# Thraix/VoxelRayTracer

Measured on AMD Instinct MI355X. Metric: Mrays/sec + achieved HBM GB/s, 1920x1080 @ 128^3 voxels, 4 bounces, higher is better.
Workload: dtype f32

## Files before the change

### voxelraytracer_amd/csrc/vrt_render.hip

```cpp
#include <hip/hip_ext.h>
#include <hip/hip_runtime.h>

#include <algorithm>
#include <cmath>
#include <cstdint>
#include <cstdio>
#include <cstring>
#include <string>
#include <vector>

#include "vrt.h"
#include "vrt_internal.h"
#include "vrt_diag.h"
#include "vrt_math.h"
#include "vrt_walk.h"
#include "vrt_cert.h"
#include "vrt_aux_kernels.h"
#include "vrt_skipfield_kernels.h"

namespace vrt {

__device__ __forceinline__ uint32_t unorm8(float f) {
  const float c = __builtin_fminf(__builtin_fmaxf(f, 0.0f), 1.0f);
  return uint32_t(__builtin_rintf(c * 255.0f));
}
__device__ __forceinline__ float unorm8_read(uint32_t b) {
  const float a = float(b), y = 1.0f / 255.0f;
  const float q0 = a * y;
  return __builtin_fmaf(__builtin_fmaf(-255.0f, q0, a), y, q0);
}
__device__ __forceinline__ uint32_t pack_rgb8(float r, float g, float b) {
  return unorm8(r) | (unorm8(g) << 8) | (unorm8(b) << 16) | 0xFF000000u;
}
__device__ __forceinline__ uint32_t temporal_blend(uint32_t nw, uint32_t old, float alpha) {
  const float om = 1.0f - alpha;
  uint32_t r = 0xFF000000u;
#pragma unroll
  for (int ch = 0; ch < 3; ++ch) {
    const float v = alpha * unorm8_read((nw >> (8 * ch)) & 0xFFu) + om * unorm8_read((old >> (8 * ch)) & 0xFFu);
    r |= unorm8(v) << (8 * ch);
  }
  return r;
}

__device__ __forceinline__ uint32_t lane_id() {
  uint32_t l;
  asm volatile("v_mbcnt_lo_u32_b32 %0, -1, 0\n\tv_mbcnt_hi_u32_b32 %0, -1, %0" : "=v"(l));
  return l;
}

__device__ __forceinline__ uint32_t* ord_ctr(const KArgs& a, uint32_t set, uint32_t r) {
  return a.order + (set * kOrdClasses + r) * kOrdCtrStride;
}
__device__ __forceinline__ uint32_t* ord_rank(const KArgs& a, uint32_t set) {
  return a.order + kOrdHdr + (1u + set) * a.tiles;
}
__device__ __forceinline__ uint32_t* ord_list(const KArgs& a, uint32_t set) {
  return a.order + kOrdHdr + 3u * a.tiles + set * (a.tiles + kOrdClasses);
}
__device__ __forceinline__ uint32_t ordered_tile(const KArgs& a, uint32_t L) {
  const uint32_t cap = kOrdClasses * a.ord_q;
  if (L < cap) {
    const uint32_t r = L % kOrdClasses, j = L / kOrdClasses;
    if (j == 0u && threadIdx.x == 0u) *ord_ctr(a, a.ctr_z, r) = 0u;
    const uint32_t n = min(*ord_ctr(a, a.ctr_r, r), a.ord_q);
    return j < n ? ord_list(a, a.ord_r)[(n - 1u - j) * kOrdClasses + r] : ~0u;
  }
  const uint32_t t = L - cap;
  return ord_rank(a, a.ord_r)[t] - 1u < a.ord_q ? ~0u : t;
}
__device__ __forceinline__ void order_record(const KArgs& a, uint32_t tile, bool heavy_wave) {
  uint32_t* cnt = a.order + kOrdHdr + tile;
  const uint32_t add = 1u | (heavy_wave ? 0x100u : 0u);
  const uint32_t old = atomicAdd(cnt, add);
  if ((old & 0xFFu) != uint32_t(kWgWaves) - 1u) return;
  *cnt = 0u;
  uint32_t rank = 0u;
  if (((old + add) & 0xFF00u) != 0u) {
    const uint32_t r = tile % kOrdClasses;
    const uint32_t k = atomicAdd(ord_ctr(a, a.ctr_w, r), 1u);
    ord_list(a, a.ord_w)[k * kOrdClasses + r] = tile;
    rank = k + 1u;
  }
  ord_rank(a, a.ord_w)[tile] = rank;
}

__device__ __forceinline__ int pixel_x(uint32_t tx, int wave, uint32_t lane) {
  return int(tx) * kTileW + (wave & 1) * 8 + int(lane & 7u);
}
__device__ __forceinline__ int pixel_row(uint32_t ty, int wave, uint32_t lane) {
  return int(ty) * kTileH + (wave >> 1) * 8 + int(lane >> 3);
}
__device__ __forceinline__ int frame_row(const KArgs& a, int li) {
  return a.row0 + (li >> a.row_blk_sh) * a.row_step + (li & ((1 << a.row_blk_sh) - 1));
}


struct FrameView {
  const float* pv;
  float time;
  uint32_t* cur;
  uint32_t* raw;
};
__device__ __forceinline__ FrameView frame_view(const KArgs& a, uint32_t f) {
  if (f == 0u) return FrameView{a.inv_pv, a.time, a.cur, a.raw};
  const KArgs::FrameB& b = a.fb[f - 1u];
  return FrameView{b.inv_pv, b.time, b.cur, b.raw};
}

template <bool LATE = false>
__device__ __forceinline__ void init_ctx(Ctx& c, const KArgs& a, const uint16_t* __restrict__ vox) {
  c.vox = vox;
  c.ostride = a.ostride;
  c.n = a.n;
  c.p = uint32_t(a.n) + 1u;
  c.fn = a.fn;
  c.max_len = a.max_len;
  c.time = a.time;
  c.refl_noise = a.refl_noise;
  c.refr_noise = a.refr_noise;
  if constexpr (LATE) {
    c.sky_sy = 0.0f;
    c.sun_n = c.sun_rcp = mk(0.0f, 0.0f, 0.0f);
    c.atlas = nullptr;
    c.atlas_mask = 0u;
    c.atlas_fs = c.atlas_fts = 0.0f;
  } else {
    c.sky_sy = a.sky_sy;
    c.sun_n = mk(a.sun_n[0], a.sun_n[1], a.sun_n[2]);
    c.sun_rcp = mk(a.sun_rcp[0], a.sun_rcp[1], a.sun_rcp[2]);
    c.atlas = a.atlas;
    c.atlas_mask = uint32_t(a.atlas_size) - 1u;
    c.atlas_fs = float(a.atlas_size);
    c.atlas_fts = float(a.atlas_tex_size);
  }
  CTRACE_ONLY(c.tr = false;)
}

__device__ __forceinline__ bool markstein_safe(float x) {
  const float m = __builtin_fabsf(x);
  return m >= 0x1p-60f && m <= 0x1p60f;
}
__device__ __forceinline__ f3 div3_rn(float x, float y, float z, float d) {
  if (markstein_safe(x) && markstein_safe(y) && markstein_safe(z) && markstein_safe(d)) {
    const float r = rcp_newton(d);
    return mk(div_rn(x, d, r), div_rn(y, d, r), div_rn(z, d, r));
  }
  return mk(x / d, y / d, z / d);
}
__device__ __forceinline__ f3 div3_lean(float x, float y, float z, float d, float r, bool rest) {
  const bool safe = rest & (__builtin_fminf(__builtin_fminf(__builtin_fabsf(x), __builtin_fabsf(y)), __builtin_fabsf(z)) >=
                            0x1p-60f);
  if (safe) return mk(div_rn(x, d, r), div_rn(y, d, r), div_rn(z, d, r));
  return mk(x / d, y / d, z / d);
}
__device__ __forceinline__ bool div3_lean_ranges(float x, float y, float z, float d) {
  return int(__builtin_fabsf(x) <= 0x1p60f) & int(__builtin_fabsf(y) <= 0x1p60f) & int(__builtin_fabsf(z) <= 0x1p60f) &
         int(markstein_safe(d));
}

template <bool LEAN = false>
__device__ __forceinline__ Ray primary_ray(const KArgs& a, const float* __restrict__ inv_pv, const Ctx& c, int px,
                                           int py) {
  const float ndx = div_rn(2.0f * (float(px) + 0.5f), LEAN ? a.fw : float(a.width), a.rcp_w) - 1.0f;
  const float ndy = div_rn(2.0f * (float(py) + 0.5f), LEAN ? a.fh : float(a.height), a.rcp_h) - 1.0f;
  float n4[4], f4[4];
#pragma unroll
  for (int i = 0; i < (LEAN ? 3 : 4); ++i) {
    const float base = inv_pv[0 * 4 + i] * ndx + inv_pv[1 * 4 + i] * ndy;
    n4[i] = (base + inv_pv[2 * 4 + i] * -1.0f) + inv_pv[3 * 4 + i] * 1.0f;
    f4[i] = (base + inv_pv[2 * 4 + i] * 1.0f) + inv_pv[3 * 4 + i] * 1.0f;
  }
  f3 vnear, vdir;
  if constexpr (LEAN) {
    float rn, rf;
    bool rest_n = true, rest_f = true;
    if ((a.setup & kSetupW) != 0u) {
      n4[3] = a.wn;
      f4[3] = a.wf;
      rn = a.rcp_wn;
      rf = a.rcp_wf;
    } else {
      const float base = inv_pv[0 * 4 + 3] * ndx + inv_pv[1 * 4 + 3] * ndy;
      n4[3] = (base + inv_pv[2 * 4 + 3] * -1.0f) + inv_pv[3 * 4 + 3] * 1.0f;
      f4[3] = (base + inv_pv[2 * 4 + 3] * 1.0f) + inv_pv[3 * 4 + 3] * 1.0f;
      if (a.vdiv_ok == 0u) {
        rest_n = div3_lean_ranges(n4[0], n4[1], n4[2], n4[3]);
        rest_f = div3_lean_ranges(f4[0], f4[1], f4[2], f4[3]);
      }
      rn = rcp_newton(n4[3]);
      rf = rcp_newton(f4[3]);
    }
    vnear = div3_lean(n4[0], n4[1], n4[2], n4[3], rn, rest_n);
    vdir = div3_lean(f4[0], f4[1], f4[2], f4[3], rf, rest_f) - vnear;
  } else {
    vnear = div3_rn(n4[0], n4[1], n4[2], n4[3]);
    vdir = div3_rn(f4[0], f4[1], f4[2], f4[3]) - vnear;
  }
  Ray ray;
  const float half_n = LEAN ? a.half_n : c.fn * 0.5f;
  ray.pos = mk(vnear.x + half_n, vnear.y + half_n, vnear.z + half_n);
  f3 dir0;
  if constexpr (LEAN) {
    const float s = vdir.x * vdir.x + vdir.y * vdir.y + vdir.z * vdir.z;
    float inv;
    if ((a.setup & kSetupLen) != 0u)
      inv = rcp_newton(sqrt_fix(s));
    else
      inv = normalize3_scale(s);
    dir0 = vdir * inv;
  } else {
    dir0 = normalize3(vdir);
  }
  ray.dir = randomize<LEAN>(dir0, vnear, a.ray_noise, c.time);
  ray.len = 0.0f;
  ray.energy = 1.0f;
  ray.voxel = 0;
  ray.rdepth = 0;
  ray.tdepth = 0;
  return ray;
}

constexpr int kStackPrio = 3;

struct StackRay {
  f3 pos, dir;
  float len, energy;
  uint32_t depths;
};
__device__ __forceinline__ StackRay pack_stack_ray(const Ray& r) {
  return StackRay{r.pos, r.dir, r.len, r.energy, uint32_t(r.rdepth) | (uint32_t(r.tdepth) << 16)};
}
constexpr int kStackWords = 9;
template <int NL>
__device__ __forceinline__ void lds_stack_put(float* __restrict__ b, const StackRay& e) {
  b[0 * NL] = e.pos.x;
  b[1 * NL] = e.pos.y;
  b[2 * NL] = e.pos.z;
  b[3 * NL] = e.dir.x;
  b[4 * NL] = e.dir.y;
  b[5 * NL] = e.dir.z;
  b[6 * NL] = e.len;
  b[7 * NL] = e.energy;
  b[8 * NL] = __uint_as_float(e.depths);
}
template <int NL>
__device__ __forceinline__ StackRay lds_stack_get(const float* __restrict__ b) {
  return StackRay{mk(b[0 * NL], b[1 * NL], b[2 * NL]), mk(b[3 * NL], b[4 * NL], b[5 * NL]), b[6 * NL],
                  b[7 * NL], __float_as_uint(b[8 * NL])};
}
__device__ __forceinline__ Ray unpack_stack_ray(const StackRay& e) {
  Ray r;
  r.pos = e.pos;
  r.dir = e.dir;
  r.len = e.len;
  r.energy = e.energy;
  r.voxel = 0;
  r.rdepth = int32_t(e.depths & 0xffffu);
  r.tdepth = int32_t(e.depths >> 16);
  return r;
}

template <bool STATS, bool TEX, bool CSH = false, bool CSEC = false, int NL = kWgThreads>
__device__ __forceinline__ bool exact_pixel(const KArgs& a, const Ctx& c, Ray ray, f3& color,
                                            Counters& k, uint32_t& steps, uint32_t& flags,
                                            int32_t& hit_vidx, float& hit_len, float* __restrict__ lstk,
                                            float s_init = -1.0f) {
  StackRay stack[kMaxStack - 2];
  const int cap = a.max_refl + a.max_transp + 1;
  int sp = 0;
  const Hit h0 = trace_with_shadow<STATS, TEX, true, CSH>(c, ray, color, k, steps, flags, s_init);
  STAMP_PIXEL_BEGIN();
  hit_vidx = h0.found ? h0.vidx : -1;
  hit_len = h0.found ? h0.len : 0.0f;
  if (h0.found && mat_id(h0.voxel) == 2) {
    __builtin_amdgcn_s_setprio(kStackPrio);
    Hit h = h0;
    for (;;) {
      Ctx lc = c;
      asm volatile("" : "+s"(lc.sun_n.x), "+s"(lc.sun_n.y), "+s"(lc.sun_n.z), "+s"(lc.sun_rcp.x),
                   "+s"(lc.sun_rcp.y), "+s"(lc.sun_rcp.z));
      bool push_r = false, push_t = false;
      if (h.found) {
        const uint32_t m = mat_id(h.voxel);
        const bool pr = mat_reflective(m) && ray.rdepth < a.max_refl;
        const bool pt = mat_transparent(m) && ray.tdepth < a.max_transp && get_color<TEX>(lc, h).w != 1.0f;
        push_r = pr && sp < cap;
        push_t = pt && sp + int(push_r) < cap;
        if ((pr && !push_r) || (pt && !push_t)) flags |= VRT_HIT_FLAG_STACK_FULL;
      }
      if (push_r && push_t) {
        const StackRay e = pack_stack_ray(reflection_ray(lc, ray, h));
        if (sp == 0)
          lds_stack_put<NL>(lstk, e);
        else
          stack[sp - 1] = e;
        ++sp;
        ray = refraction_ray<TEX>(lc, ray, h, k);
      } else if (push_r) {
        ray = reflection_ray(lc, ray, h);
      } else if (push_t) {
        ray = refraction_ray<TEX>(lc, ray, h, k);
      } else {
        if (sp == 0) break;
        --sp;
        ray = unpack_stack_ray(sp == 0 ? lds_stack_get<NL>(lstk) : stack[sp - 1]);
      }
      k.c[VRT_CNT_SECONDARY_RAYS]++;
      if constexpr (CSH && CSEC) {
        bool settled;
        h = march_cert(lc, ray, color, settled, k, steps, flags);
        if (settled) {
          h.found = false;
          continue;
        }
        shade<STATS, TEX, CSH>(lc, ray, h, color, k, steps, flags);
        continue;
      }
      h = trace_with_shadow<STATS, TEX, false, CSH>(lc, ray, color, k, steps, flags);
    }
    STAMP_PIXEL_END();
    return true;
  }
  return false;
}

template <class KA>
__device__ __forceinline__ void store_pixel(const KA& a, const FrameView& fv, float4* __restrict__ out,
                                            size_t o, const f3 color) {
  if (fv.cur) {
    const uint32_t rw = pack_rgb8(color.x, color.y, color.z);
    if (fv.raw) fv.raw[o] = rw;
    fv.cur[o] = a.alpha == 1.0f ? rw : temporal_blend(rw, a.prev[o], a.alpha);
  } else {
    out[o] = make_float4(color.x, color.y, color.z, 1.0f);
  }
}

template <bool STATS, bool TEX, int CERT = 0, bool ORD = false, bool DEFER = false, bool FB = false,
          bool TREE = false>
__global__ void __launch_bounds__(kWgThreads, TREE ? kTreeWaves : (DEFER ? kDeferWaves : kMinWaves)) render_kernel(KArgs a, const uint16_t* __restrict__ vox,
                                                     float4* __restrict__ out,
                                                     vrt_hit* __restrict__ hits,
                                                     unsigned long long* __restrict__ counters) {
  const int wave = __builtin_amdgcn_readfirstlane(int(threadIdx.x) >> 6);
  STAMP_WAVE_BEGIN(wave);
  uint32_t tile = 0u;
  uint32_t fr = 0u, tx, ty;
  if constexpr (DEFER) {
    static_assert(!ORD, "the certified pass has no tile order");
    tx = blockIdx.x;
    ty = blockIdx.y;
    if constexpr (FB) fr = blockIdx.z;
  } else {
    tile = blockIdx.x;
    if constexpr (ORD) {
      tile = ordered_tile(a, blockIdx.x);
      if (tile == ~0u) return;
    }
    tile = __builtin_amdgcn_readfirstlane(tile);
    if constexpr (FB) fr = uint32_t(__builtin_amdgcn_readfirstlane(int(tile / a.frame_tiles)));
    const uint32_t ltile = tile - fr * a.frame_tiles;
    ty = ltile / a.tiles_x;
    tx = ltile - ty * a.tiles_x;
  }
  const int px = pixel_x(tx, wave, lane_id());
  const int li = pixel_row(ty, wave, lane_id());
  const bool valid = px < a.width && li < a.rows;
  bool heavy = false;
  bool deferred = false;

  Counters k;
#pragma unroll
  for (int q = 0; q < VRT_CNT_COUNT; ++q) k.c[q] = 0;

  if (valid) {
    Ctx c;
    init_ctx<DEFER>(c, a, vox);
    CTRACE_ONLY(c.tr = px == VRT_TRACE_PX && frame_row(a, li) == VRT_TRACE_PY;)
    if constexpr (FB) c.time = frame_view(a, fr).time;
    constexpr int kAxFloats = DEFER && !TREE ? 0 : kWgThreads * 3 * 4;
    constexpr int kStkFloats = std::max(DEFER ? 0 : kStackWords * kWgThreads,
                                        TREE ? (kTreeWords - 12) * kWgThreads : 0);
    constexpr int kPool = std::max(kAxFloats + kStkFloats, 4);
    __shared__ float4 lds_pool[kPool / 4];
    c.ax = &lds_pool[threadIdx.x * kAxLane];
    const Ray ray = primary_ray<DEFER>(a, FB ? frame_view(a, fr).pv : a.inv_pv, c, px, frame_row(a, li));
    k.c[VRT_CNT_PIXELS] = 1;
    k.c[VRT_CNT_PRIMARY_RAYS] = 1;
    uint32_t steps = 0, flags = 0;
    int32_t hit_vidx = -1;
    float hit_len = 0.0f;
    f3 color;
    if constexpr (!DEFER) color = mk(0.0f, 0.0f, 0.0f);
    float* tstk = nullptr;
    if constexpr (TREE) {
      static_assert(CERT == 2 && !TEX && !STATS, "certified trees: stats-free colour-only certified instances");
      tstk = reinterpret_cast<float*>(lds_pool) + kAxFloats + threadIdx.x;
    }
    float us = -1.0f;
    bool need_exact;
    if (DEFER && (PHASE_STOP(0) || PHASE_STOP(1))) {
      color = PHASE_STOP(1) ? mk(ray.pos.x + ray.dir.x, ray.pos.y + ray.dir.y, ray.pos.z + ray.dir.z)
                            : mk(0.0f, 0.0f, 0.0f);
      need_exact = false;
    } else {
      need_exact = CERT < 2 || !cert_pixel<TEX, TREE, kWgThreads, DEFER>(c, ray, color, a.max_refl, a.max_transp, tstk, &us, &a);
    }
    STAMP_WAVE_CERT(need_exact);
    if constexpr (DEFER) {
      deferred = need_exact;
    } else if (need_exact) {
      color = mk(0.0f, 0.0f, 0.0f);
      heavy = true;
      float* lstk = reinterpret_cast<float*>(lds_pool) + kAxFloats;
      (void)exact_pixel<STATS, TEX, CERT >= 1, CERT == 2>(a, c, ray, color, k, steps, flags, hit_vidx,
                                                         hit_len, &lstk[threadIdx.x], STATS ? -1.0f : us);
    }
    const uint32_t l2 = lane_id();
    const size_t o = size_t(pixel_row(ty, wave, l2)) * size_t(a.pitch) + size_t(pixel_x(tx, wave, l2));
    if (STATS && hits) {
      vrt_hit hr;
      hr.voxel_index = hit_vidx;
      hr.ray_length = hit_len;
      hr.steps = steps;
      hr.flags = flags;
      hits[o] = hr;
    }
    if constexpr (DEFER) {
      if (!deferred) {
        LateKArgs* ka = late_kargs();
        uint32_t *cur = ka->cur, *raw = ka->raw;
        if (FB && fr != 0u) {
          cur = ka->fb[fr - 1u].cur;
          raw = ka->fb[fr - 1u].raw;
        }
        store_pixel(*ka, FrameView{nullptr, 0.0f, cur, raw}, out, o, color);
      }
    } else {
      if (!deferred) store_pixel(a, FB ? frame_view(a, fr) : FrameView{a.inv_pv, a.time, a.cur, a.raw}, out, o, color);
    }
  }
  if constexpr (DEFER) {
    const unsigned long long m = __ballot(deferred);
    if (m != 0ull) {
      const uint32_t seg = tx * kOrdClasses / a.tiles_x;
      const uint32_t first = uint32_t(__builtin_ctzll(m));
      const uint32_t cnt = uint32_t(__builtin_popcountll(m));
      const bool dense = cnt >= kDeferDense;
      uint32_t base = 0;
      if (lane_id() == first)
        base = atomicAdd(a.defer + ((uint32_t(dense) * 2u + a.defer_e) * kOrdClasses + seg) * kOrdCtrStride,
                         dense ? 1u : cnt);
      base = uint32_t(__builtin_amdgcn_readlane(int(base), int(first)));
      uint32_t* list = a.defer + kDeferHdr + seg * a.defer_seg;
      const uint32_t l3 = lane_id();
      const uint32_t id = (fr << 29) | (uint32_t(pixel_row(ty, wave, l3)) << 16) | uint32_t(pixel_x(tx, wave, l3));
      if (dense) {
        list[a.defer_seg - 64u * (base + 1u) + l3] = deferred ? id : ~0u;
      } else if (deferred) {
        const uint32_t rank = __builtin_amdgcn_mbcnt_hi(uint32_t(m >> 32), __builtin_amdgcn_mbcnt_lo(uint32_t(m), 0u));
        list[base + rank] = id;
      }
    }
  }
  if constexpr (ORD) {
    const bool heavy_wave = __ballot(heavy) != 0ull;
    if (lane_id() == 0) order_record(a, tile, heavy_wave);
  }
  STAMP_WAVE_END();
  if (STATS && counters) {
    unsigned long long* slot = counters + size_t(blockIdx.x % kCntReplicas) * VRT_CNT_COUNT;
#pragma unroll
    for (int q = 0; q < VRT_CNT_COUNT; ++q) {
      unsigned long long v = k.c[q];
#pragma unroll
      for (int off = 32; off > 0; off >>= 1) v += __shfl_xor(v, off, 64);
      if (lane_id() == 0 && v) atomicAdd(slot + q, v);
    }
  }
}

template <bool TEX, int CERT, int WAVES = kExactWaves, uint32_t SB = kSparseBatch, bool FB = false>
__global__ void __launch_bounds__(64, WAVES) exact_pass_kernel(KArgs a, const uint16_t* __restrict__ vox,
                                                                     float4* __restrict__ out) {
  const uint32_t* ctr = a.defer;
  if (blockIdx.x == 0 && threadIdx.x < 2u * kOrdClasses) {
    const uint32_t l = threadIdx.x;
    a.defer[(((l / kOrdClasses) * 2u + (a.defer_e ^ 1u)) * kOrdClasses + l % kOrdClasses) * kOrdCtrStride] = 0u;
  }
  uint32_t ns[kOrdClasses], nd[kOrdClasses], total_s = 0, total_d = 0;
#pragma unroll
  for (uint32_t q = 0; q < kOrdClasses; ++q) {
    ns[q] = uint32_t(__builtin_amdgcn_readfirstlane(int(ctr[(a.defer_e * kOrdClasses + q) * kOrdCtrStride])));
    nd[q] = uint32_t(__builtin_amdgcn_readfirstlane(int(ctr[((2u + a.defer_e) * kOrdClasses + q) * kOrdCtrStride])));
    total_s += ns[q];
    total_d += nd[q];
  }
  static_assert(SB >= 1 && SB <= 64, "lanes SB.. of a sparse batch idle");
  const uint32_t batches = total_d + (total_s + SB - 1u) / SB;
  if (a.batches_out && blockIdx.x == 0 && threadIdx.x == 0)
    *a.batches_out = batches;
  if (blockIdx.x >= batches) return;
  if constexpr (kExactPrio > 0) __builtin_amdgcn_s_setprio(kExactPrio);
  const uint32_t lane = lane_id();
  STAMP_PASS_BEGIN();
  Ctx c;
  init_ctx(c, a, vox);
  __shared__ float4 ax_tab[64 * 3];
  c.ax = &ax_tab[lane * kAxLane];
  for (uint32_t b = blockIdx.x; b < batches; b += gridDim.x) {
    const bool dense = b < total_d;
    uint32_t idx = dense ? b : (b - total_d) * SB + lane;
    if (!dense && (lane >= SB || idx >= total_s)) continue;
    uint32_t seg = 0;
#pragma unroll
    for (uint32_t q = 0; q + 1u < kOrdClasses; ++q) {
      const uint32_t nq = dense ? nd[q] : ns[q];
      const bool past = seg == q && idx >= nq;
      idx -= past ? nq : 0u;
      seg += past ? 1u : 0u;
    }
    const uint32_t* list = a.defer + kDeferHdr + seg * a.defer_seg;
    const uint32_t e = dense ? list[a.defer_seg - 64u * (idx + 1u) + lane] : list[idx];
    if (e == ~0u) continue;
    Ray ray;
    if constexpr (FB) {
      const FrameView fv = frame_view(a, e >> 29);
      c.time = fv.time;
      ray = primary_ray(a, fv.pv, c, int(e & 0xFFFFu), frame_row(a, int((e >> 16) & 0x1FFFu)));
    } else {
      ray = primary_ray(a, a.inv_pv, c, int(e & 0xFFFFu), frame_row(a, int(e >> 16)));
    }
    Counters k;
#pragma unroll
    for (int q = 0; q < VRT_CNT_COUNT; ++q) k.c[q] = 0;
    uint32_t steps = 0, flags = 0;
    int32_t hit_vidx = -1;
    float hit_len = 0.0f;
    f3 color = mk(0.0f, 0.0f, 0.0f);
    __shared__ float lstk[kStackWords * 64];
    (void)exact_pixel<false, TEX, CERT >= 1, CERT == 2 && !TEX, 64>(a, c, ray, color, k, steps, flags,
                                                                    hit_vidx, hit_len, &lstk[lane]);
    if constexpr (FB) {
      uint32_t e2 = e;
      asm volatile("" : "+v"(e2));
      store_pixel(a, frame_view(a, e2 >> 29), out,
                  size_t((e2 >> 16) & 0x1FFFu) * size_t(a.pitch) + size_t(e2 & 0xFFFFu), color);
    } else {
      store_pixel(a, FrameView{a.inv_pv, a.time, a.cur, a.raw}, out,
                  size_t(e >> 16) * size_t(a.pitch) + size_t(e & 0xFFFFu), color);
    }
    STAMP_PASS_BATCH(dense);
  }
  STAMP_PASS_END(lane);
}

}

#include "vrt_query_kernels.h"
#include "vrt_trace_kernels.h"
#include "vrt_ids_kernels.h"
#include "vrt_reproject_kernels.h"

namespace vrt {


static unsigned grid_blocks(uint64_t items) { return unsigned(std::min<uint64_t>((items + 255) / 256, 16384)); }

void launch_render(const KArgs& a, bool stats, const uint16_t* vox, float4* out, vrt_hit* hit,
                   unsigned long long* cnt_rep, hipStream_t s, hipEvent_t ev_begin, hipEvent_t ev_end) {
  const dim3 grid(a.order ? kOrdClasses * a.ord_q + a.tiles : a.tiles);
  if (a.defer && !stats && a.cert == 2) {
    const dim3 g1(a.tiles_x, a.frame_tiles / a.tiles_x, uint32_t(a.nframes)),
        g2(a.exact_grid ? a.exact_grid
                        : std::max(64u, a.tiles * uint32_t(kWgWaves) / (a.textured ? kDeferGridDiv : kDeferGridDivColor)));
    const bool fb = a.nframes > 1;
    auto k1 = a.textured ? (fb ? render_kernel<false, true, 2, false, true, true> : render_kernel<false, true, 2, false, true>)
              : a.tree   ? (fb ? render_kernel<false, false, 2, false, true, true, true>
                               : render_kernel<false, false, 2, false, true, false, true>)
                         : (fb ? render_kernel<false, false, 2, false, true, true> : render_kernel<false, false, 2, false, true>);
    auto k2 = a.textured ? (fb ? exact_pass_kernel<true, 1, kExactWaves, kSparseBatchTex, true>
                               : exact_pass_kernel<true, 1, kExactWaves, kSparseBatchTex>)
                         : (a.exact_fat
                                ? (fb ? exact_pass_kernel<false, 2, kFatWaves, kSparseBatchFat, true>
                                      : exact_pass_kernel<false, 2, kFatWaves, kSparseBatchFat>)
                                : (fb ? exact_pass_kernel<false, 2, kExactWaves, kSparseBatch, true>
                                      : exact_pass_kernel<false, 2>));
    const uint32_t pad = a.tree ? 0u : kDeferLdsPad;
    if (ev_begin)
      hipExtLaunchKernelGGL(k1, g1, dim3(kWgThreads), pad, s, ev_begin, nullptr, 0, a, vox, out, hit, cnt_rep);
    else
      hipLaunchKernelGGL(k1, g1, dim3(kWgThreads), pad, s, a, vox, out, hit, cnt_rep);
    if (ev_end)
      hipExtLaunchKernelGGL(k2, g2, dim3(64), 0, s, nullptr, ev_end, 0, a, vox, out);
    else
      hipLaunchKernelGGL(k2, g2, dim3(64), 0, s, a, vox, out);
    return;
  }
  auto kern = a.textured ? (stats ? render_kernel<true, true>
                            : a.nframes > 1 ? (a.cert >= 1 ? render_kernel<false, true, 1, false, false, true>
                                                           : render_kernel<false, true, 0, false, false, true>)
                                            : (a.cert >= 1 ? render_kernel<false, true, 1> : render_kernel<false, true>))
                         : (stats ? render_kernel<true, false>
                            : a.nframes > 1
                                ? (a.cert == 2 ? (a.order ? render_kernel<false, false, 2, true, false, true>
                                                          : render_kernel<false, false, 2, false, false, true>)
                                   : a.cert == 1 ? render_kernel<false, false, 1, false, false, true>
                                                 : render_kernel<false, false, 0, false, false, true>)
                                : (a.cert == 2 ? (a.tree ? (a.order ? render_kernel<false, false, 2, true, false, false, true>
                                                                    : render_kernel<false, false, 2, false, false, false, true>)
                                                 : a.order ? render_kernel<false, false, 2, true>
                                                           : render_kernel<false, false, 2>)
                                   : a.cert == 1 ? render_kernel<false, false, 1>
                                                 : render_kernel<false, false, 0>));
  if (ev_begin || ev_end)
    hipExtLaunchKernelGGL(kern, grid, dim3(kWgThreads), 0, s, ev_begin, ev_end, 0, a, vox, out, hit, cnt_rep);
  else
    hipLaunchKernelGGL(kern, grid, dim3(kWgThreads), 0, s, a, vox, out, hit, cnt_rep);
}

void launch_ray_query(const KArgs& a, int32_t kind, const uint16_t* vox, const void* in, uint32_t count,
                      vrt_ray_hit* hits, hipStream_t s, hipEvent_t ev_begin, hipEvent_t ev_end) {
  auto kern = kind == kQueryPick           ? ray_query_kernel<kQueryPick>
              : kind == VRT_CAST_OCCLUSION ? ray_query_kernel<VRT_CAST_OCCLUSION>
                                           : ray_query_kernel<VRT_CAST_NEAREST>;
  const dim3 grid((count + uint32_t(kQueryWg) - 1u) / uint32_t(kQueryWg));
  if (ev_begin || ev_end)
    hipExtLaunchKernelGGL(kern, grid, dim3(kQueryWg), 0, s, ev_begin, ev_end, 0, a, vox, in, count,
                          reinterpret_cast<uint4*>(hits));
  else
    hipLaunchKernelGGL(kern, grid, dim3(kQueryWg), 0, s, a, vox, in, count, reinterpret_cast<uint4*>(hits));
}

void launch_ray_trace(const KArgs& a, int32_t kind, const uint16_t* vox, const void* in, uint32_t count,
                      vrt_ray_color* out, hipStream_t s, hipEvent_t ev_begin, hipEvent_t ev_end) {
  auto kern = kind == kTracePixels
                  ? (a.textured ? ray_trace_kernel<kTracePixels, true> : ray_trace_kernel<kTracePixels, false>)
                  : (a.textured ? ray_trace_kernel<kTraceRays, true> : ray_trace_kernel<kTraceRays, false>);
  const dim3 grid((count + uint32_t(kTraceWg) - 1u) / uint32_t(kTraceWg));
  if (ev_begin || ev_end)
    hipExtLaunchKernelGGL(kern, grid, dim3(kTraceWg), 0, s, ev_begin, ev_end, 0, a, vox, in, count,
                          reinterpret_cast<uint4*>(out));
  else
    hipLaunchKernelGGL(kern, grid, dim3(kTraceWg), 0, s, a, vox, in, count, reinterpret_cast<uint4*>(out));
}

void launch_render_ids(const KArgs& a, const uint16_t* vox, vrt_pixel_id* ids, float* depth, hipStream_t s,
                       hipEvent_t ev_begin, hipEvent_t ev_end) {
  const dim3 grid(uint32_t(a.width + 7) / 8u, uint32_t(a.rows + 7) / 8u);
  if (ev_begin || ev_end)
    hipExtLaunchKernelGGL(ids_exact_kernel, grid, dim3(64), 0, s, ev_begin, ev_end, 0, a, vox,
                          reinterpret_cast<uint2*>(ids), depth);
  else
    hipLaunchKernelGGL(ids_exact_kernel, grid, dim3(64), 0, s, a, vox, reinterpret_cast<uint2*>(ids), depth);
}

void launch_reproject(const KArgs& a, const ReprojArgs& r, hipStream_t s, hipEvent_t ev_begin, hipEvent_t ev_end) {
  const dim3 grid(uint32_t(a.width + 15) / 16u, uint32_t(a.rows + 15) / 16u);
  if (ev_begin || ev_end)
    hipExtLaunchKernelGGL(reproject_kernel, grid, dim3(kReprojWg), 0, s, ev_begin, ev_end, 0, a, r);
  else
    hipLaunchKernelGGL(reproject_kernel, grid, dim3(kReprojWg), 0, s, a, r);
}

void launch_reproject_fetch(const KArgs& a, const ReprojArgs& r, int32_t fetch, uint8_t* taps, hipStream_t s,
                            hipEvent_t ev_begin, hipEvent_t ev_end) {
  if (fetch == VRT_FETCH_NEAREST && !taps) return launch_reproject(a, r, s, ev_begin, ev_end);
  auto kern = fetch == VRT_FETCH_BILINEAR ? reproject_bilinear_kernel : reproject_nearest_taps_kernel;
  const dim3 grid(uint32_t(a.width + 15) / 16u, uint32_t(a.rows + 15) / 16u);
  if (ev_begin || ev_end)
    hipExtLaunchKernelGGL(kern, grid, dim3(kReprojWg), 0, s, ev_begin, ev_end, 0, a, r, taps);
  else
    hipLaunchKernelGGL(kern, grid, dim3(kReprojWg), 0, s, a, r, taps);
}

void launch_reduce_counters(unsigned long long* rep, unsigned long long* dst, hipStream_t s) {
  hipLaunchKernelGGL(reduce_counters_kernel, dim3(1), dim3(64), 0, s, rep, dst);
}

namespace {

struct Span {
  int32_t a, b;
};
Span clip_span(int64_t a, int64_t b, int32_t n) {
  return Span{int32_t(std::max<int64_t>(a, 0)), int32_t(std::min<int64_t>(b, int64_t(n) - 1))};
}
Span fwd_anchors(int32_t lo, int32_t hi, int sg, int32_t n) {
  const int64_t r = int64_t(kFwdCap) - 1;
  return sg > 0 ? clip_span(lo - r, int64_t(hi) - 1, n) : clip_span(lo, int64_t(hi) - 1 + r, n);
}
Span fwd_inputs(int32_t lo, int32_t hi, int32_t n) {
  const int64_t r = int64_t(kFwdCap) - 1;
  return clip_span(lo - r, int64_t(hi) - 1 + r, n);
}
Span fwd_texels(int32_t lo, int32_t hi, int sg, int32_t n) {
  const int64_t r = int64_t(kFwdCap) - 1;
  const int64_t a = (sg > 0 ? lo - r : int64_t(lo)) + sg, b = (sg > 0 ? int64_t(hi) - 1 : int64_t(hi) - 1 + r) + sg;
  return clip_span(std::min<int64_t>(a, lo), std::max<int64_t>(b, int64_t(hi) - 1), n);
}
Span dist_span(int32_t lo, int32_t hi, int64_t reach, int32_t n) {
  return clip_span(lo - reach, int64_t(hi) - 1 + reach, n);
}
Region region_of(Span x, Span y, Span z) {
  return Region{x.a, y.a, z.a, x.b - x.a + 1, y.b - y.a + 1, z.b - z.a + 1};
}

}

int volume_edit_plan(int32_t n, int octants, const int32_t lo[3], const int32_t ext[3], int32_t* out) {
  for (int o = 0; o < octants; ++o)
    for (int a = 0; a < 3; ++a) {
      const int32_t hi = lo[a] + ext[a];
      const Span t = octants == 8 ? fwd_texels(lo[a], hi, (o >> a & 1) ? -1 : 1, n)
                                  : dist_span(lo[a], hi, int64_t(kDistCap) - 1, n);
      out[o * 6 + a] = t.a;
      out[o * 6 + 3 + a] = t.b + 1;
    }
  return octants;
}

void launch_edit_apply(const uint8_t* box, uint8_t* vox, uint32_t n, const int32_t lo[3], const int32_t ext[3],
                       unsigned long long* counts, hipStream_t s) {
  const Region b{lo[0], lo[1], lo[2], ext[0], ext[1], ext[2]};
  hipLaunchKernelGGL(edit_apply_kernel, dim3(grid_blocks(region_cells(b))), dim3(256), 0, s, box, vox, b, n,
                     counts);
}

void launch_volume_edit_passes(const uint8_t* vox, uint8_t* tmp, uint16_t* packed, uint32_t n, int octants,
                               const int32_t lo[3], const int32_t ext[3], bool distances, hipStream_t s) {
  const int32_t ni = int32_t(n);
  const int32_t hi[3] = {lo[0] + ext[0], lo[1] + ext[1], lo[2] + ext[2]};
  const uint64_t vol = uint64_t(n) * n * n, pvol = uint64_t(n + 1) * (n + 1) * (n + 1);
  const Region box{lo[0], lo[1], lo[2], ext[0], ext[1], ext[2]};
  const Region whole{0, 0, 0, ni, ni, ni};
  uint8_t* da = tmp;
  uint8_t* db = tmp + vol;
  if (octants == 8) {
    uint8_t* dc = tmp + 2 * vol;
    const Span iy = fwd_inputs(lo[1], hi[1], ni), iz = fwd_inputs(lo[2], hi[2], ni);
    for (int sx = 1; sx >= -1; sx -= 2) {
      const Span ax = fwd_anchors(lo[0], hi[0], sx, ni);
      const Region rx = region_of(ax, iy, iz);
      if (distances)
        hipLaunchKernelGGL(fwd_pass_kernel, dim3(grid_blocks(region_cells(rx))), dim3(256), 0, s, vox,
                           whole, da, rx, n, 0, sx, 1);
      for (int sy = 1; sy >= -1; sy -= 2) {
        const Span ay = fwd_anchors(lo[1], hi[1], sy, ni);
        const Region ry = region_of(ax, ay, iz);
        if (distances)
          hipLaunchKernelGGL(fwd_pass_kernel, dim3(grid_blocks(region_cells(ry))), dim3(256), 0, s, da,
                             rx, db, ry, n, 1, sy, 0);
        for (int sz = 1; sz >= -1; sz -= 2) {
          const Span az = fwd_anchors(lo[2], hi[2], sz, ni);
          const Region rz = region_of(ax, ay, az);
          const int o = (sx < 0 ? 1 : 0) | (sy < 0 ? 2 : 0) | (sz < 0 ? 4 : 0);
          uint16_t* dst = packed + size_t(o) * pvol;
          if (distances) {
            hipLaunchKernelGGL(fwd_pass_kernel, dim3(grid_blocks(region_cells(rz))), dim3(256), 0, s, db,
                               ry, dc, rz, n, 2, sz, 0);
            const Region pb = region_of(fwd_texels(lo[0], hi[0], sx, ni), fwd_texels(lo[1], hi[1], sy, ni),
                                        fwd_texels(lo[2], hi[2], sz, ni));
            hipLaunchKernelGGL(fwd_pack_kernel, dim3(grid_blocks(region_cells(pb))), dim3(256), 0, s, vox,
                               dc, rz, dst, pb, n, sx, sy, sz);
          } else {
            hipLaunchKernelGGL(fwd_pack_kernel, dim3(grid_blocks(region_cells(box))), dim3(256), 0, s, vox,
                               static_cast<const uint8_t*>(nullptr), box, dst, box, n, sx, sy, sz);
          }
        }
      }
    }
  } else if (distances) {
    const int64_t r1 = int64_t(kDistCap) - 1;
    const Span ax = dist_span(lo[0], hi[0], r1, ni), ay = dist_span(lo[1], hi[1], r1, ni);
    const Span az = dist_span(lo[2], hi[2], r1, ni);
    const Span iy = dist_span(lo[1], hi[1], 2 * r1, ni), iz = dist_span(lo[2], hi[2], 2 * r1, ni);
    const Region rx = region_of(ax, iy, iz), ry = region_of(ax, ay, iz), rz = region_of(ax, ay, az);
    hipLaunchKernelGGL(dist_pass_kernel, dim3(grid_blocks(region_cells(rx))), dim3(256), 0, s, vox, whole,
                       da, rx, n, 0, 1);
    hipLaunchKernelGGL(dist_pass_kernel, dim3(grid_blocks(region_cells(ry))), dim3(256), 0, s, da, rx, db,
                       ry, n, 1, 0);
    hipLaunchKernelGGL(dist_pass_kernel, dim3(grid_blocks(region_cells(rz))), dim3(256), 0, s, db, ry, da,
                       rz, n, 2, 0);
    hipLaunchKernelGGL(pack_volume_kernel, dim3(grid_blocks(region_cells(rz))), dim3(256), 0, s, vox, da,
                       rz, packed, rz, n);
  } else {
    hipLaunchKernelGGL(pack_volume_kernel, dim3(grid_blocks(region_cells(box))), dim3(256), 0, s, vox,
                       static_cast<const uint8_t*>(nullptr), box, packed, box, n);
  }
  const int wrap = (lo[0] == 0 ? 1 : 0) | (lo[1] == 0 ? 2 : 0) | (lo[2] == 0 ? 4 : 0);
  if (wrap) {
    const EdgeSlabs e = edge_slabs(box, wrap);
    hipLaunchKernelGGL(edge_pack_kernel, dim3(grid_blocks(e.cz + e.cy + e.cx)), dim3(256), 0, s, vox, packed, pvol,
                       octants, box, wrap, n);
  }
}

void launch_glass_share(const uint8_t* vox, uint64_t total, unsigned long long* out, hipStream_t s) {
  hipLaunchKernelGGL(glass_share_kernel, dim3(grid_blocks(total)), dim3(256), 0, s, vox, total, out);
}

void launch_build_scene(uint8_t* vox, int scene, uint32_t n, const float* noise, hipStream_t s) {
  const uint64_t vol = uint64_t(n) * n * n;
  hipLaunchKernelGGL(build_scene_kernel, dim3(grid_blocks(vol)), dim3(256), 0, s, vox, scene, n, noise);
}

void launch_assemble_blocks(const uint32_t* bands, uint64_t band_words, int32_t k, int32_t sh, int32_t width,
                            int32_t height, uint32_t* frame, uint64_t frame_pitch, hipStream_t s) {
  if (height <= 0 || width <= 0) return;
  const bool vec = width % 4 == 0 && band_words % 4 == 0 && frame_pitch % 4 == 0 &&
                   (reinterpret_cast<uintptr_t>(bands) & 15u) == 0 && (reinterpret_cast<uintptr_t>(frame) & 15u) == 0;
  if (vec)
    hipLaunchKernelGGL(assemble_blocks_kernel<true>, dim3(uint32_t(height)), dim3(256), 0, s, bands, band_words, k,
                       sh, width, frame, frame_pitch);
  else
    hipLaunchKernelGGL(assemble_blocks_kernel<false>, dim3(uint32_t(height)), dim3(256), 0, s, bands, band_words, k,
                       sh, width, frame, frame_pitch);
}

void launch_pack_rgb8(const uint32_t* rgba, uint64_t pixels, uint8_t* rgb, hipStream_t s) {
  const uint64_t quads = pixels / 4u;
  if (quads == 0) return;
  hipLaunchKernelGGL(pack_rgb8_kernel, dim3(grid_blocks(quads)), dim3(256), 0, s, reinterpret_cast<const uint4*>(rgba), quads,
                     reinterpret_cast<uint32_t*>(rgb));
}

void launch_assemble_blocks_rgb8(const uint8_t* bands, uint64_t band_px, int32_t k, int32_t sh, int32_t width,
                                 int32_t height, uint32_t* frame, uint64_t frame_pitch, hipStream_t s) {
  if (height <= 0 || width <= 0) return;
  hipLaunchKernelGGL(assemble_blocks_rgb8_kernel, dim3(uint32_t(height)), dim3(256), 0, s,
                     reinterpret_cast<const uint32_t*>(bands), band_px, k, sh, width, reinterpret_cast<uint4*>(frame),
                     frame_pitch);
}

int run_fast_math_check(unsigned long long* host_out) {
  unsigned long long* d = nullptr;
  if (hipMalloc(&d, 7 * sizeof(unsigned long long)) != hipSuccess) return VRT_ERR_OOM;
  const unsigned long long init[7] = {0, 0, 0, 0, ~0ull, 0, 0};
  hipError_t e = hipMemcpy(d, init, sizeof(init), hipMemcpyHostToDevice);
  if (e == hipSuccess) {
    hipLaunchKernelGGL(fast_math_check_kernel, dim3(1u << 16), dim3(256), 0, nullptr, d);
    e = hipGetLastError();
  }
  if (e == hipSuccess) e = hipMemcpy(host_out, d, sizeof(init), hipMemcpyDeviceToHost);
  (void)hipFree(d);
  return e == hipSuccess ? VRT_OK : VRT_ERR_DEVICE;
}

void launch_randomize(const float* dir, const float* pos, int n, float randomness, float seed,
                      float* out, hipStream_t s) {
  hipLaunchKernelGGL(randomize_kernel, dim3((n + 63) / 64), dim3(64), 0, s, dir, pos, n,
                     randomness, seed, out);
}

}
```

### voxelraytracer_amd/csrc/vrt_tuning.h

```cpp
#ifndef VRT_TUNING_H
#define VRT_TUNING_H

#include <cstdint>

#if (defined(VRT_MIN_WAVES) || defined(VRT_DEFER_WAVES) || defined(VRT_EXACT_WAVES) || defined(VRT_TREE_WAVES) || \
     defined(VRT_FAT_WAVES) || defined(VRT_SPARSE_BATCH) || defined(VRT_SPARSE_BATCH_TEX) ||                    \
     defined(VRT_SPARSE_BATCH_FAT) || defined(VRT_EXACT_PRIO) || defined(VRT_FWD_CAP) || defined(VRT_WG_WAVES) || \
     defined(VRT_ORD_DIV) || defined(VRT_ORD_MIN_ROUNDS) || defined(VRT_DEFER_GRID_DIV) ||                      \
     defined(VRT_DEFER_GRID_DIV_COLOR) || defined(VRT_QUERY_WG_WAVES) || defined(VRT_TRACE_WG_WAVES) ||         \
     defined(VRT_TRACE_MIN_WAVES) || defined(VRT_DEFER_LDS_PAD)) &&                                                                         \
    !defined(VRT_DIAGNOSTIC_BUILD)
#error "the VRT_* tuning values are A/B knobs of make variant builds (make variant NAME=... DEFS=-DVRT_...=...)"
#endif

#ifndef VRT_WG_WAVES
#define VRT_WG_WAVES 2
#endif
#ifndef VRT_MIN_WAVES
#define VRT_MIN_WAVES 7
#endif
#ifndef VRT_DEFER_WAVES
#define VRT_DEFER_WAVES 7
#endif
#ifndef VRT_DEFER_LDS_PAD
#define VRT_DEFER_LDS_PAD 0
#endif
#ifndef VRT_EXACT_WAVES
#define VRT_EXACT_WAVES VRT_MIN_WAVES
#endif
#ifndef VRT_TREE_WAVES
#define VRT_TREE_WAVES 5
#endif
#ifndef VRT_FAT_WAVES
#define VRT_FAT_WAVES 3
#endif
#ifndef VRT_SPARSE_BATCH
#define VRT_SPARSE_BATCH 32
#endif
#ifndef VRT_SPARSE_BATCH_TEX
#define VRT_SPARSE_BATCH_TEX 64
#endif
#ifndef VRT_SPARSE_BATCH_FAT
#define VRT_SPARSE_BATCH_FAT 16
#endif
#ifndef VRT_EXACT_PRIO
#define VRT_EXACT_PRIO 2
#endif
#ifndef VRT_FWD_CAP
#define VRT_FWD_CAP 128
#endif
#ifndef VRT_ORD_DIV
#define VRT_ORD_DIV 4
#endif
#ifndef VRT_ORD_MIN_ROUNDS
#define VRT_ORD_MIN_ROUNDS 1
#endif
#ifndef VRT_DEFER_GRID_DIV
#define VRT_DEFER_GRID_DIV 8
#endif
#ifndef VRT_DEFER_GRID_DIV_COLOR
#define VRT_DEFER_GRID_DIV_COLOR VRT_DEFER_GRID_DIV
#endif
#ifndef VRT_QUERY_WG_WAVES
#define VRT_QUERY_WG_WAVES 1
#endif
#ifndef VRT_TRACE_WG_WAVES
#define VRT_TRACE_WG_WAVES 1
#endif
#ifndef VRT_TRACE_MIN_WAVES
#define VRT_TRACE_MIN_WAVES 6
#endif

namespace vrt {

constexpr int kWgWaves = VRT_WG_WAVES;
static_assert(kWgWaves == 1 || kWgWaves == 2 || kWgWaves == 4, "1, 2 or 4 waves per workgroup");

constexpr int kMinWaves = VRT_MIN_WAVES;
constexpr int kDeferWaves = VRT_DEFER_WAVES;
constexpr uint32_t kDeferLdsPad = VRT_DEFER_LDS_PAD;
constexpr int kExactWaves = VRT_EXACT_WAVES;
constexpr int kTreeWaves = VRT_TREE_WAVES;
constexpr int kFatWaves = VRT_FAT_WAVES;

constexpr uint32_t kSparseBatch = VRT_SPARSE_BATCH;
constexpr uint32_t kSparseBatchTex = VRT_SPARSE_BATCH_TEX;
constexpr uint32_t kSparseBatchFat = VRT_SPARSE_BATCH_FAT;
constexpr int kExactPrio = VRT_EXACT_PRIO;

constexpr uint32_t kFwdCap = VRT_FWD_CAP;
static_assert(kFwdCap >= 3 && kFwdCap <= 255, "F and G are stored in 8 bits");

constexpr uint32_t kOrdDiv = VRT_ORD_DIV;
constexpr uint32_t kOrdMinRounds = VRT_ORD_MIN_ROUNDS;
constexpr uint32_t kDeferGridDiv = VRT_DEFER_GRID_DIV;
constexpr uint32_t kDeferGridDivColor = VRT_DEFER_GRID_DIV_COLOR;

constexpr int kQueryWgWaves = VRT_QUERY_WG_WAVES;
static_assert(kQueryWgWaves >= 1 && kQueryWgWaves <= 4, "1 to 4 waves per query workgroup");
constexpr int kTraceWgWaves = VRT_TRACE_WG_WAVES;
static_assert(kTraceWgWaves >= 1 && kTraceWgWaves <= 4, "1 to 4 waves per trace workgroup");
constexpr int kTraceMinWaves = VRT_TRACE_MIN_WAVES;

}

#endif
```

Before: 106,700.

## Cap exact-pass VGPRs and reload kernel args late from kernarg segment

Adds a VGPR-capped variant of the untextured exact-pass kernel, now the default, with a 120-register cap. The kernel reads KArgs straight from the kernarg segment. In the untextured path it re-fetches context, depth limits, defer counters and store pointers from kernel args at the point of use instead of keeping them live. The aim is to cut register pressure so more waves fit per SIMD, at the cost of extra scalar loads and possible spills if the cap is too tight.

```diff
diff --git a/voxelraytracer_amd/csrc/vrt_render.hip b/voxelraytracer_amd/csrc/vrt_render.hip
--- a/voxelraytracer_amd/csrc/vrt_render.hip
+++ b/voxelraytracer_amd/csrc/vrt_render.hip
@@ -261,15 +261,24 @@
   return r;
 }
 
-template <bool STATS, bool TEX, bool CSH = false, bool CSEC = false, int NL = kWgThreads>
+template <bool STATS, bool TEX, bool CSH = false, bool CSEC = false, int NL = kWgThreads, bool LATE = false>
 __device__ __forceinline__ bool exact_pixel(const KArgs& a, const Ctx& c, Ray ray, f3& color,
                                             Counters& k, uint32_t& steps, uint32_t& flags,
                                             int32_t& hit_vidx, float& hit_len, float* __restrict__ lstk,
                                             float s_init = -1.0f) {
+  static_assert(!LATE || !TEX, "a textured walk reads the atlas");
   StackRay stack[kMaxStack - 2];
-  const int cap = a.max_refl + a.max_transp + 1;
+  const int cap0 = LATE ? 0 : a.max_refl + a.max_transp + 1;
   int sp = 0;
-  const Hit h0 = trace_with_shadow<STATS, TEX, true, CSH>(c, ray, color, k, steps, flags, s_init);
+  Hit h0;
+  if constexpr (LATE) {
+    h0 = march<STATS, TEX, true>(c, ray, k, steps, flags, s_init);
+    Ctx lc = c;
+    late_ctx(lc);
+    shade<STATS, TEX, CSH>(lc, ray, h0, color, k, steps, flags);
+  } else {
+    h0 = trace_with_shadow<STATS, TEX, true, CSH>(c, ray, color, k, steps, flags, s_init);
+  }
   STAMP_PIXEL_BEGIN();
   hit_vidx = h0.found ? h0.vidx : -1;
   hit_len = h0.found ? h0.len : 0.0f;
@@ -278,13 +287,25 @@
     Hit h = h0;
     for (;;) {
       Ctx lc = c;
-      asm volatile("" : "+s"(lc.sun_n.x), "+s"(lc.sun_n.y), "+s"(lc.sun_n.z), "+s"(lc.sun_rcp.x),
-                   "+s"(lc.sun_rcp.y), "+s"(lc.sun_rcp.z));
+      int max_refl, max_transp, cap;
+      if constexpr (LATE) {
+        late_ctx(lc);
+        LateKArgs* ka = late_kargs();
+        max_refl = ka->max_refl;
+        max_transp = ka->max_transp;
+        cap = max_refl + max_transp + 1;
+      } else {
+        asm volatile("" : "+s"(lc.sun_n.x), "+s"(lc.sun_n.y), "+s"(lc.sun_n.z), "+s"(lc.sun_rcp.x),
+                     "+s"(lc.sun_rcp.y), "+s"(lc.sun_rcp.z));
+        max_refl = a.max_refl;
+        max_transp = a.max_transp;
+        cap = cap0;
+      }
       bool push_r = false, push_t = false;
       if (h.found) {
         const uint32_t m = mat_id(h.voxel);
-        const bool pr = mat_reflective(m) && ray.rdepth < a.max_refl;
-        const bool pt = mat_transparent(m) && ray.tdepth < a.max_transp && get_color<TEX>(lc, h).w != 1.0f;
+        const bool pr = mat_reflective(m) && ray.rdepth < max_refl;
+        const bool pt = mat_transparent(m) && ray.tdepth < max_transp && get_color<TEX>(lc, h).w != 1.0f;
         push_r = pr && sp < cap;
         push_t = pt && sp + int(push_r) < cap;
         if ((pr && !push_r) || (pt && !push_t)) flags |= VRT_HIT_FLAG_STACK_FULL;
@@ -481,9 +502,10 @@
   }
 }
 
-template <bool TEX, int CERT, int WAVES = kExactWaves, uint32_t SB = kSparseBatch, bool FB = false>
-__global__ void __launch_bounds__(64, WAVES) exact_pass_kernel(KArgs a, const uint16_t* __restrict__ vox,
-                                                                     float4* __restrict__ out) {
+template <bool TEX, int CERT, uint32_t SB, bool FB>
+__device__ __forceinline__ void exact_pass_body(const KArgs& a, const uint16_t* __restrict__ vox,
+                                                float4* __restrict__ out) {
+  constexpr bool LATE = !TEX;
   const uint32_t* ctr = a.defer;
   if (blockIdx.x == 0 && threadIdx.x < 2u * kOrdClasses) {
     const uint32_t l = threadIdx.x;
@@ -506,23 +528,38 @@
   const uint32_t lane = lane_id();
   STAMP_PASS_BEGIN();
   Ctx c;
-  init_ctx(c, a, vox);
+  init_ctx<LATE>(c, a, vox);
   __shared__ float4 ax_tab[64 * 3];
   c.ax = &ax_tab[lane * kAxLane];
   for (uint32_t b = blockIdx.x; b < batches; b += gridDim.x) {
     const bool dense = b < total_d;
     uint32_t idx = dense ? b : (b - total_d) * SB + lane;
     if (!dense && (lane >= SB || idx >= total_s)) continue;
-    uint32_t seg = 0;
+    uint32_t seg = 0, e;
+    if constexpr (LATE) {
+      LateKArgs* kq = late_kargs();
+      const uint32_t kind = uint32_t(__builtin_amdgcn_readfirstlane(dense ? 2 : 0));
+      const uint32_t* cq = kq->defer + (kind + kq->defer_e) * kOrdClasses * kOrdCtrStride;
 #pragma unroll
-    for (uint32_t q = 0; q + 1u < kOrdClasses; ++q) {
-      const uint32_t nq = dense ? nd[q] : ns[q];
-      const bool past = seg == q && idx >= nq;
-      idx -= past ? nq : 0u;
-      seg += past ? 1u : 0u;
-    }
-    const uint32_t* list = a.defer + kDeferHdr + seg * a.defer_seg;
-    const uint32_t e = dense ? list[a.defer_seg - 64u * (idx + 1u) + lane] : list[idx];
+      for (uint32_t q = 0; q + 1u < kOrdClasses; ++q) {
+        const uint32_t nq = uint32_t(__builtin_amdgcn_readfirstlane(int(cq[q * kOrdCtrStride])));
+        const bool past = seg == q && idx >= nq;
+        idx -= past ? nq : 0u;
+        seg += past ? 1u : 0u;
+      }
+      const uint32_t* list = kq->defer + kDeferHdr + seg * kq->defer_seg;
+      e = dense ? list[kq->defer_seg - 64u * (idx + 1u) + lane] : list[idx];
+    } else {
+#pragma unroll
+      for (uint32_t q = 0; q + 1u < kOrdClasses; ++q) {
+        const uint32_t nq = dense ? nd[q] : ns[q];
+        const bool past = seg == q && idx >= nq;
+        idx -= past ? nq : 0u;
+        seg += past ? 1u : 0u;
+      }
+      const uint32_t* list = a.defer + kDeferHdr + seg * a.defer_seg;
+      e = dense ? list[a.defer_seg - 64u * (idx + 1u) + lane] : list[idx];
+    }
     if (e == ~0u) continue;
     Ray ray;
     if constexpr (FB) {
@@ -540,20 +577,55 @@
     float hit_len = 0.0f;
     f3 color = mk(0.0f, 0.0f, 0.0f);
     __shared__ float lstk[kStackWords * 64];
-    (void)exact_pixel<false, TEX, CERT >= 1, CERT == 2 && !TEX, 64>(a, c, ray, color, k, steps, flags,
-                                                                    hit_vidx, hit_len, &lstk[lane]);
-    if constexpr (FB) {
-      uint32_t e2 = e;
-      asm volatile("" : "+v"(e2));
-      store_pixel(a, frame_view(a, e2 >> 29), out,
-                  size_t((e2 >> 16) & 0x1FFFu) * size_t(a.pitch) + size_t(e2 & 0xFFFFu), color);
+    (void)exact_pixel<false, TEX, CERT >= 1, CERT == 2 && !TEX, 64, LATE>(a, c, ray, color, k, steps, flags,
+                                                                          hit_vidx, hit_len, &lstk[lane]);
+    uint32_t e2 = e;
+    if constexpr (FB || LATE) asm volatile("" : "+v"(e2));
+    const uint32_t row = FB ? (e2 >> 16) & 0x1FFFu : e2 >> 16;
+    if constexpr (LATE) {
+      LateKArgs* ka = late_kargs();
+      uint32_t *cur = ka->cur, *raw = ka->raw;
+      if constexpr (FB) {
+        const uint32_t f = e2 >> 29;
+        if (f != 0u) {
+          cur = ka->fb[f - 1u].cur;
+          raw = ka->fb[f - 1u].raw;
+        }
+      }
+      store_pixel(*ka, FrameView{nullptr, 0.0f, cur, raw}, out, size_t(row) * size_t(ka->pitch) + size_t(e2 & 0xFFFFu),
+                  color);
     } else {
-      store_pixel(a, FrameView{a.inv_pv, a.time, a.cur, a.raw}, out,
-                  size_t(e >> 16) * size_t(a.pitch) + size_t(e & 0xFFFFu), color);
+      store_pixel(a, FB ? frame_view(a, e2 >> 29) : FrameView{a.inv_pv, a.time, a.cur, a.raw}, out,
+                  size_t(row) * size_t(a.pitch) + size_t(e2 & 0xFFFFu), color);
     }
     STAMP_PASS_BATCH(dense);
   }
   STAMP_PASS_END(lane);
+}
+
+__device__ __forceinline__ const KArgs& kernel_kargs() {
+  return *(const KArgs*)__builtin_amdgcn_kernarg_segment_ptr();
+}
+template <bool TEX, int CERT, int WAVES = kExactWaves, uint32_t SB = kSparseBatch, bool FB = false>
+__global__ void __launch_bounds__(64, WAVES) exact_pass_kernel(KArgs ,
+                                                               const uint16_t* __restrict__ vox,
+                                                               float4* __restrict__ out) {
+  exact_pass_body<TEX, CERT, SB, FB>(kernel_kargs(), vox, out);
+}
+template <int CERT, uint32_t SB, bool FB>
+__global__ void __launch_bounds__(64, exact_cap_waves(kExactVgprs))
+    __attribute__((amdgpu_num_vgpr(exact_cap_attr(kExactVgprs))))
+    exact_pass_kernel_capped(KArgs , const uint16_t* __restrict__ vox,
+                             float4* __restrict__ out) {
+  exact_pass_body<false, CERT, SB, FB>(kernel_kargs(), vox, out);
+}
+using ExactPassFn = void (*)(KArgs, const uint16_t*, float4*);
+template <int CAP>
+static ExactPassFn exact_pass_whole_frame(bool fb) {
+  if constexpr (CAP == 0)
+    return fb ? exact_pass_kernel<false, 2, kExactWaves, kSparseBatch, true> : exact_pass_kernel<false, 2>;
+  else
+    return fb ? exact_pass_kernel_capped<2, kSparseBatch, true> : exact_pass_kernel_capped<2, kSparseBatch, false>;
 }
 
 }
@@ -580,13 +652,11 @@
               : a.tree   ? (fb ? render_kernel<false, false, 2, false, true, true, true>
                                : render_kernel<false, false, 2, false, true, false, true>)
                          : (fb ? render_kernel<false, false, 2, false, true, true> : render_kernel<false, false, 2, false, true>);
-    auto k2 = a.textured ? (fb ? exact_pass_kernel<true, 1, kExactWaves, kSparseBatchTex, true>
-                               : exact_pass_kernel<true, 1, kExactWaves, kSparseBatchTex>)
-                         : (a.exact_fat
-                                ? (fb ? exact_pass_kernel<false, 2, kFatWaves, kSparseBatchFat, true>
-                                      : exact_pass_kernel<false, 2, kFatWaves, kSparseBatchFat>)
-                                : (fb ? exact_pass_kernel<false, 2, kExactWaves, kSparseBatch, true>
-                                      : exact_pass_kernel<false, 2>));
+    ExactPassFn k2 = a.textured ? (fb ? exact_pass_kernel<true, 1, kExactWaves, kSparseBatchTex, true>
+                                      : exact_pass_kernel<true, 1, kExactWaves, kSparseBatchTex>)
+                     : a.exact_fat ? (fb ? exact_pass_kernel<false, 2, kFatWaves, kSparseBatchFat, true>
+                                         : exact_pass_kernel<false, 2, kFatWaves, kSparseBatchFat>)
+                                   : exact_pass_whole_frame<kExactVgprs>(fb);
     const uint32_t pad = a.tree ? 0u : kDeferLdsPad;
     if (ev_begin)
       hipExtLaunchKernelGGL(k1, g1, dim3(kWgThreads), pad, s, ev_begin, nullptr, 0, a, vox, out, hit, cnt_rep);
diff --git a/voxelraytracer_amd/csrc/vrt_tuning.h b/voxelraytracer_amd/csrc/vrt_tuning.h
--- a/voxelraytracer_amd/csrc/vrt_tuning.h
+++ b/voxelraytracer_amd/csrc/vrt_tuning.h
@@ -8,7 +8,7 @@
      defined(VRT_SPARSE_BATCH_FAT) || defined(VRT_EXACT_PRIO) || defined(VRT_FWD_CAP) || defined(VRT_WG_WAVES) || \
      defined(VRT_ORD_DIV) || defined(VRT_ORD_MIN_ROUNDS) || defined(VRT_DEFER_GRID_DIV) ||                      \
      defined(VRT_DEFER_GRID_DIV_COLOR) || defined(VRT_QUERY_WG_WAVES) || defined(VRT_TRACE_WG_WAVES) ||         \
-     defined(VRT_TRACE_MIN_WAVES) || defined(VRT_DEFER_LDS_PAD)) &&                                                                         \
+     defined(VRT_TRACE_MIN_WAVES) || defined(VRT_DEFER_LDS_PAD) || defined(VRT_EXACT_VGPRS)) &&                 \
     !defined(VRT_DIAGNOSTIC_BUILD)
 #error "the VRT_* tuning values are A/B knobs of make variant builds (make variant NAME=... DEFS=-DVRT_...=...)"
 #endif
@@ -27,6 +27,9 @@
 #endif
 #ifndef VRT_EXACT_WAVES
 #define VRT_EXACT_WAVES VRT_MIN_WAVES
+#endif
+#ifndef VRT_EXACT_VGPRS
+#define VRT_EXACT_VGPRS 120
 #endif
 #ifndef VRT_TREE_WAVES
 #define VRT_TREE_WAVES 5
@@ -80,6 +83,11 @@
 constexpr int kDeferWaves = VRT_DEFER_WAVES;
 constexpr uint32_t kDeferLdsPad = VRT_DEFER_LDS_PAD;
 constexpr int kExactWaves = VRT_EXACT_WAVES;
+constexpr int kExactVgprs = VRT_EXACT_VGPRS;
+static_assert(kExactVgprs == 0 || (kExactVgprs >= 64 && kExactVgprs <= 256 && kExactVgprs % 8 == 0),
+              "a VGPR cap of 64 to 256 in whole allocation granules, or 0 for none");
+constexpr int exact_cap_waves(int v) { return v > 0 ? 512 / ((v + 7) / 8 * 8) : 1; }
+constexpr int exact_cap_attr(int v) { return v > 0 ? v / 2 : 256; }
 constexpr int kTreeWaves = VRT_TREE_WAVES;
 constexpr int kFatWaves = VRT_FAT_WAVES;
 
```

New measurement: 113,300, median of 6. +6.2%, better.
